# mmechtley/psfMC

Measured on AMD Instinct MI355X. Metric: walker log-posterior evals/sec, 256x256 image, 1 PSF+1 Sersic, higher is better.
Workload: dtype f64

## Files before the change

psfmc_amd/csrc/psfmc_fused_path.h:

```cpp
#pragma once
#ifndef PSFMC_PART
#define PSFMC_PART 0
#endif
#include "psfmc_device.h"
#include "psfmc_fft.h"

#ifndef PSFMC_COLS3G_MIN
#define PSFMC_COLS3G_MIN 0
#endif

namespace psfmc {

#ifndef PSFMC_ROW_WAVES
#define PSFMC_ROW_WAVES 0
#endif
constexpr int kColThreads = 256;
#ifndef PSFMC_COLS_PRIO
#define PSFMC_COLS_PRIO 3
#endif
#ifndef PSFMC_INV_PRIO
#define PSFMC_INV_PRIO 0
#endif
#ifndef PSFMC_INV_REMAP_MIN
#define PSFMC_INV_REMAP_MIN 720
// ... 111 lines not shown
__device__ __forceinline__ int t_elem(int y, int c, int rg_log2) {
    const int rg = 1 << rg_log2;
    return (((y >> rg_log2) * 2 + c) << rg_log2) + (y & (rg - 1));
}
#ifndef PSFMC_T_PAD
#define PSFMC_T_PAD 0
#endif
__host__ __device__ __forceinline__ int t_col_len(int ny, int rg_log2) {
    const int len = ((ny + (1 << rg_log2) - 1) >> rg_log2) << rg_log2;
    return (PSFMC_T_PAD && (len & 127) == 0) ? len + (1 << rg_log2) : len;
}

struct FieldPx {
    double sci, var;
};

template <int NX> constexpr size_t fused_field_len(int ny) {
    return (size_t)((ny + FftShape<NX>::TPW - 1) / FftShape<NX>::TPW) * FftShape<NX>::R * 64;
}

template <int NX>
__global__ void k_pack_field(const double* __restrict__ sci, const double* __restrict__ obs_var,
                             const uint8_t* __restrict__ bad, FieldPx* __restrict__ out, int ny) {
    using S = FftShape<NX>;
    constexpr int T = S::T, R = S::R, RG = S::TPW;
    const int n = (int)fused_field_len<NX>(ny);
    for (int i = blockIdx.x * blockDim.x + threadIdx.x; i < n; i += gridDim.x * blockDim.x) {
        const int lane = i & 63, e = (i >> 6) % R, yg = i / (64 * R);
        const int f = lane / T, t = lane % T;
        const int y = yg * RG + f, x = fft_k_of<NX>(t, e);
        const bool holds = f < RG && y < ny && fft_slot_valid<NX>(t, e);
        const size_t src = holds ? (size_t)y * NX + x : 0;
        out[i] = holds ? FieldPx{bad[src] ? __builtin_nan("") : sci[src], obs_var[src]}
                       : FieldPx{__builtin_nan(""), 1.0};
    }
}

template <int NX, bool FROM_IMAGE, typename TS = cd, bool FAST = FftShape<NX>::kPlain, bool WRAP = false,
          bool EXTRA = false>
__global__ void __launch_bounds__((row_threads<NX, FAST>()), (fused_row_min_waves<NX, false, WRAP>()))
k_rows_fwd(const double* __restrict__ prep, const uint8_t* __restrict__ skip,
           const cd* __restrict__ twx, TS* __restrict__ Tbuf, int n_ps, int n_sersic, int ny,
           int ps_only, const double* __restrict__ img, const double* __restrict__ img_scale,
           double* __restrict__ raw_out, const WrapDesc* __restrict__ wrap_tab, int pow_mode) {
    using S = FftShape<NX>;
    constexpr int P = S::P, T = S::T, R = S::R, RG = row_group<NX>();
    constexpr int NXH = NX / 2 + 1;
    constexpr int RGL2 = layout_rg_log2<NX, FAST>(), RGL = 1 << RGL2;
    extern __shared__ __align__(16) double smem[];
// ... 624 lines not shown
template <class S> constexpr bool cols3f_half_table() { return cols3f_waves<S>() == 8; }
template <class S> constexpr int cols3f_table_rows() { return cols3f_half_table<S>() ? S::R1 / 2 : S::R1; }
template <class S> constexpr size_t fused_col3f_lds_used() {
    return ((size_t)cols3f_waves<S>() * fft3g_lds_doubles<S>() + (size_t)cols3f_table_rows<S>() * 64 * 2) * sizeof(double);
}
template <class S> constexpr size_t fused_col3f_lds_bytes() { return fused_col3f_lds_used<S>(); }
#ifndef PSFMC_COLS3F_PREFETCH
#define PSFMC_COLS3F_PREFETCH -1
#endif
#ifndef PSFMC_COLS3F_WAVES16
#define PSFMC_COLS3F_WAVES16 3
#endif
template <class S> constexpr bool cols3f_prefetch() {
    return PSFMC_COLS3F_PREFETCH < 0 ? (S::R1 == 16 || (S::R1 == 32 && !cols3f_half_table<S>())) : PSFMC_COLS3F_PREFETCH != 0;
}
template <class S> constexpr int cols3f_min_waves() {
    if (cols3f_prefetch<S>()) return S::R1 <= 8 ? 3 : S::R1 <= 16 ? 2 : 1;
    return S::R1 <= 8 ? 4 : S::R1 <= 16 ? PSFMC_COLS3F_WAVES16 : (S::R1 <= 24 || cols3f_half_table<S>()) ? 2 : 1;
}

template <int NY, bool CONVOLVE, class S = Fft3gShape<NY>>
__global__ void __launch_bounds__((cols3f_threads<S>()), (cols3f_min_waves<S>()))
k_cols3f(cd* __restrict__ Tbuf, const cd* __restrict__ Kt, const double* __restrict__ prep,
         const uint8_t* __restrict__ skip, const cd* __restrict__ twy, int plen, int nxh, int n_w, int rg_log2) {
    static_assert(cols3f_shape<S>(), "ny = 8 m x 8 x 8");
    constexpr int R1 = S::R1, NB3 = S::NB3, WPB = cols3f_waves<S>();
    constexpr bool HALF = cols3f_half_table<S>();
    static_assert(NB3 * 8 == R1, "registers");
    static_assert(fused_col3f_lds_bytes<S>() <= 160 * 1024, "a workgroup's LDS");
    extern __shared__ __align__(16) double smem[];
// ... 72 lines not shown
            }
            __builtin_amdgcn_sched_barrier(0);
            fft_wave3g<S, +1, HALF>(v, o, w2, t, lds, tab, w1h);
            __builtin_amdgcn_sched_barrier(0);
            if (live) {
                unsigned os = off_b;
                if constexpr (kScalar) asm volatile("" : "+v"(os));
#pragma unroll
                for (int q = 0; q < NB3; ++q)
#pragma unroll
                    for (int k3 = 0; k3 < 8; ++k3) *t_at(base, os, q + NB3 * k3) = o[q][k3];
            }
        }
        return;
    }
    for (int grp = gr.first; grp < gr.end; grp += gr.step) {
        const int col = grp * WPB + wave;
        if (col >= n_cols) continue;
        const int pr = col >> 1, c = col & 1;
        const int kx = __builtin_amdgcn_readfirstlane(pr / n_w), w = pr - kx * n_w;
        const bool skipped = skip && skip[w];
        cd* base = Tbuf + ((size_t)w * nxh + kx) * 2 * nyp + (c << rg_log2);
        unsigned ob = off_b, kb = kt_b;
        if constexpr (kScalar) asm volatile("" : "+v"(ob), "+v"(kb));
        cd v[R1];
#pragma unroll
        for (int a = 0; a < R1; ++a) v[a] = load_stream(t_at(base, ob, a));
        if (skipped) continue;
        cd o[NB3][8];
        fft_wave3g<S, -1, HALF>(v, o, w2, t, lds, tab, w1h);
        if constexpr (CONVOLVE) {
            __builtin_amdgcn_sched_barrier(0);
            const int psf = __builtin_amdgcn_readfirstlane((int)prep[(size_t)w * plen + kPrepPsfIdx]);
            const cd* k = Kt + (((size_t)psf * nxh + kx) * 2 + c) * NY;
#pragma unroll
            for (int q = 0; q < NB3; ++q)
#pragma unroll
                for (int k3 = 0; k3 < 8; ++k3) v[q + NB3 * k3] = cmul(o[q][k3], *k_at(k, kb, q + NB3 * k3));
            __builtin_amdgcn_sched_barrier(0);
            fft_wave3g<S, +1, HALF>(v, o, w2, t, lds, tab, w1h);
            __builtin_amdgcn_sched_barrier(0);
        }
        unsigned os = off_b;
        if constexpr (kScalar) asm volatile("" : "+v"(os));
#pragma unroll
        for (int q = 0; q < NB3; ++q)
#pragma unroll
            for (int k3 = 0; k3 < 8; ++k3) *t_at(base, os, q + NB3 * k3) = o[q][k3];
    }
}

template <int NX, typename TS = cd, bool FAST = FftShape<NX>::kPlain, bool MULTI = false>
__global__ void __launch_bounds__((row_threads<NX, FAST>()), (fused_row_min_waves<NX, true>()))
k_rows_inv(const TS* __restrict__ Tbuf, const uint8_t* __restrict__ skip, const cd* __restrict__ twx,
           const FieldPx* __restrict__ field, double* __restrict__ partial, int ny,
           const double* __restrict__ prep, int plen,
           double* __restrict__ conv_out, double* __restrict__ var_out, int n_psf_field, unsigned field_stride) {
    using S = FftShape<NX>;
    constexpr int P = S::P, T = S::T, R = S::R, RG = row_group<NX>();
    constexpr int NXH = NX / 2 + 1;
    constexpr int RGL2 = layout_rg_log2<NX, FAST>(), RGL = 1 << RGL2;
    extern __shared__ __align__(16) double smem[];
#if PSFMC_INV_PRIO
    __builtin_amdgcn_s_setprio(PSFMC_INV_PRIO);
#endif

    int w = blockIdx.y, bx = blockIdx.x;
    if constexpr (inv_remap<NX, FAST>()) {
        const int gx = (int)gridDim.x, n_w = (int)gridDim.y;
        const int id = w * gx + bx;
// ... 91 lines not shown
    load_twiddles<NX>(tw, twx, t, twl, lane);
    fft_wave<NX, +1>(v, tw, twx, t, wave_lds + (size_t)fe * fft_lds_elems<NX>(), twl, lane_on);
    const double inv_lambda = prep[(size_t)w * plen + kPrepInvLambda];

    if (conv_out) {
        const size_t rowoff = (size_t)w * ny * NX + (size_t)(row_on ? iy : 0) * NX;
#pragma unroll
        for (int e = 0; e < R; ++e) {
            if (row_on && fft_slot_valid<NX>(t, e)) {
                const int x = fft_k_of<NX>(t, e);
                conv_out[rowoff + x] = v[e].x;
                var_out[rowoff + x] = v[e].y * inv_lambda;
            }
        }
    }
    const FieldPx* fbase = field + (size_t)yg * R * 64;
    if (MULTI || (NX < 1024 && n_psf_field > 0))
        fbase += (size_t)((int)prep[(size_t)w * plen + kPrepPsfIdx] / n_psf_field) * field_stride;
    const unsigned foff = (unsigned)lane * (unsigned)sizeof(FieldPx);
    constexpr int CH = (FAST && R == 32) ? PSFMC_INV_CHUNK : R, NCH = R / CH;
    static_assert(R % CH == 0, "chunks");
    double acc = 0.0, mant = 1.0;
    int expo = 0, n_good = 0;
    bool invalid = false;
    auto load_chunk = [&](FieldPx (&px)[CH], int c) {
#pragma unroll
        for (int j = 0; j < CH; ++j) px[j] = *at_bytes(fbase, foff + (unsigned)((c * CH + j) * 64 * sizeof(FieldPx)));
    };
    auto sum_chunk = [&](const FieldPx (&px)[CH], int c) {
        bool any_bad = false;
#pragma unroll
        for (int j = 0; j < CH; ++j) any_bad |= px[j].sci != px[j].sci;
        if (!__any(any_bad)) {
#pragma unroll
            for (int j = 0; j < CH; ++j) {
                const int e = c * CH + j;
                const double d = __builtin_fma(v[e].y, inv_lambda, px[j].var);
                const double r = px[j].sci - v[e].x;
                acc = __builtin_fma(r * r, fast_rcp(d), acc);
                invalid |= !(d > 0.0);
                mant *= __builtin_amdgcn_frexp_mant(d);
                expo += __builtin_amdgcn_frexp_exp(d);
            }
            n_good += CH;
        } else {
#pragma unroll
            for (int j = 0; j < CH; ++j) {
                const int e = c * CH + j;
                const bool good = px[j].sci == px[j].sci;
                const double d = __builtin_fma(v[e].y, inv_lambda, px[j].var);
                const double r = px[j].sci - v[e].x;
                const double a1 = __builtin_fma(r * r, fast_rcp(d), acc);
                acc = good ? a1 : acc;
                const double dd = good ? d : 1.0;
                invalid |= !(dd > 0.0);
                mant *= __builtin_amdgcn_frexp_mant(dd);
                expo += __builtin_amdgcn_frexp_exp(dd);
                n_good += good ? 1 : 0;
            }
        }
    };
    if constexpr (NCH == 1) {
        FieldPx px[CH];
        load_chunk(px, 0);
        sum_chunk(px, 0);
    } else {
        static_assert(NCH % 2 == 0, "chunk pairs");
        FieldPx pa[CH], pb[CH];
        load_chunk(pa, 0);
#pragma unroll
        for (int c = 0; c < NCH; c += 2) {
            load_chunk(pb, c + 1);
            sum_chunk(pa, c);
            if (c + 2 < NCH) load_chunk(pa, c + 2);
            sum_chunk(pb, c + 1);
        }
    }
    acc += 0.69314718055994530942 * (fast_log2(mant) + (double)expo) +
           1.83787706640934548356 * (double)n_good;
    acc = invalid ? __builtin_nan("") : acc;
#pragma unroll
    for (int o = 32; o > 0; o >>= 1) acc += __shfl_down(acc, o, 64);
    if (lane == 0) partial[(size_t)w * nyg + yg] = acc;
// ... 177 lines not shown
```

psfmc_amd/csrc/psfmc_hip.hip:

```cpp
#include "../../include/psfmc_hip.h"
#include "psfmc_side_costs.h"

#ifndef PSFMC_NPARTS
#define PSFMC_NPARTS 1
#define PSFMC_PART 0
#endif

#include <hip/hip_runtime.h>
#include <hipfft/hipfft.h>

#include <cmath>
#include <cstdarg>
#include <cstdio>
#include <cstdlib>
#include <cstring>
#include <map>
#include <string>
#include <utility>
#include <vector>

#include "psfmc_device.h"
#if PSFMC_PART == 0
#include "psfmc_hipfft_path.h"
#endif
// ... 261 lines not shown
        case 1280: { constexpr int N_ = 1280; BODY; } break; \
        default: return PSFMC_NOT_MINE; \
    }
#endif

struct psfmc_ctx {
    int device = 0;
    int ny = 0, nx = 0, nxh = 0, S = 0, F = 0;
    int nyp = 0;
    bool embed = false;
    std::vector<WrapDesc> wraps;
    WrapDesc* d_wrap = nullptr;
    int n_psf = 0, n_ps = 0, n_sersic = 0;
    int n_fields = 1, n_psf_field = 0;
    size_t field_len = 0;
    int max_walkers = 0, chunk = 0, backend = 0;
    bool prep_tabs_built = false;
    bool prep_tabs_valid = false;
    bool use_pow_tabs = true;
    int single_cap = 0;
    int rlen = 0, plen = 0;
    int nblk = 0;
    hipStream_t stream = nullptr;
    double *d_sci = nullptr, *d_var = nullptr;
    uint8_t* d_bad = nullptr;
    double *d_rows = nullptr, *d_prep = nullptr, *d_like = nullptr, *d_partial = nullptr;
    uint8_t* d_skip = nullptr;
    double2 *d_pspec = nullptr, *d_vspec = nullptr;
    double* d_real = nullptr;
    double2* d_spec = nullptr;
// ... 16 lines not shown
    long long speculated_runs = 0;
    int speculate = -1;
    int cols3 = 1;
    bool use_graph = false;
    long long graph_launches = 0;
    int min_split = 1 << 30;
    bool profile = false;
    struct ProfRec { int kind; hipEvent_t a, b; };
    std::vector<ProfRec> prof_pending;
    double prof_ms[3] = {0, 0, 0};
    long prof_n[3] = {0, 0, 0};
    cd* d_Kraw = nullptr;
    cd* d_Kt = nullptr;
    cd *d_twx = nullptr, *d_twy = nullptr;
    double* d_rho = nullptr;
    FieldPx* d_field = nullptr;
    int rg_log2 = 0;
    double *d_img0 = nullptr, *d_img1 = nullptr;
    int img_cap = 0;
    bool has_layout = false;
    ThetaLayout layout{};
    std::vector<ThetaLayout> more_layouts;
    std::vector<void*> more_blobs;
    std::vector<char> more_has;
    size_t theta_lds = 0;
    ThetaLayout* d_field_layouts = nullptr;
    int* d_field_sides = nullptr;
    void* d_layout_blob = nullptr;
    struct Joint {
        bool ready = false;
        ThetaLayout prior{};
// ... 83 lines not shown
    return PSFMC_OK;
}
template <int NX, bool FROM_IMAGE>
static int launch_rows3_fwd(psfmc_ctx* c, int n, const double* prep, const uint8_t* skip, cd* Tbuf, int ps_only,
                            const double* img, const double* img_scale, double* raw_out, hipStream_t st) {
    if constexpr (!rows3_fwd_built(NX)) {
        return fail(PSFMC_EINVAL, "side %d has no three-stage row kernels", NX);
    } else {
        if constexpr (!FROM_IMAGE) {
            if (c->embed)
                return launch_rows3_fwd_kernel<NX, false, true>(c, n, prep, skip, Tbuf, ps_only, img, img_scale, raw_out, st);
        }
        return launch_rows3_fwd_kernel<NX, FROM_IMAGE, false>(c, n, prep, skip, Tbuf, ps_only, img, img_scale, raw_out, st);
    }
}
template <int NX, bool MULTI>
static int launch_rows3_inv_kernel(psfmc_ctx* c, int n, const cd* Tbuf, const double* prep, const uint8_t* skip,
                                   double* partial, double* conv_out, double* var_out, hipStream_t st) {
    using S = typename Rows3<NX>::S;
    constexpr size_t lds = rows3_lds_bytes<S>();
    if constexpr (lds > 64 * 1024) {
        static thread_local int attr_device = -1;
        if (attr_device != c->device) {
            HIP_TRY(hipFuncSetAttribute(reinterpret_cast<const void*>(&k_rows3_inv<NX, MULTI>),
                                        hipFuncAttributeMaxDynamicSharedMemorySize, (int)lds));
            attr_device = c->device;
        }
    }
    hipLaunchKernelGGL((k_rows3_inv<NX, MULTI>), dim3((c->ny + rows3_waves(NX) - 1) / rows3_waves(NX), n), dim3(rows3_threads(NX)), lds,
                       st, Tbuf, skip, c->d_twx, c->d_field, partial, c->ny, prep, c->plen, conv_out, var_out,
                       c->n_fields > 1 ? c->n_psf_field : 0, (unsigned)c->field_len);
    return PSFMC_OK;
}
template <int NX>
static int launch_rows3_inv(psfmc_ctx* c, int n, const cd* Tbuf, const double* prep, const uint8_t* skip,
                            double* partial, double* conv_out, double* var_out, hipStream_t st) {
    if constexpr (!rows3_side<NX>()) {
        return fail(PSFMC_EINVAL, "side %d has no three-stage row kernels", NX);
    } else {
        if (c->n_fields > 1) return launch_rows3_inv_kernel<NX, true>(c, n, Tbuf, prep, skip, partial, conv_out, var_out, st);
        return launch_rows3_inv_kernel<NX, false>(c, n, Tbuf, prep, skip, partial, conv_out, var_out, st);
    }
}

template <int NX, bool FROM_IMAGE, typename TS, bool FAST, bool WRAP, bool EXTRA = false>
static int launch_rows_fwd_kernel(psfmc_ctx* c, int n, const double* prep, const uint8_t* skip, TS* Tbuf,
                                  int ps_only, const double* img, const double* img_scale, double* raw_out,
                                  hipStream_t st) {
    constexpr size_t lds = fused_row_lds_bytes<NX, FAST>();
    if constexpr (!FROM_IMAGE && !EXTRA) {
        if (const double* extra = ps_only ? nullptr : integ_image_of(c, prep))
            return launch_rows_fwd_kernel<NX, false, TS, FAST, WRAP, true>(c, n, prep, skip, Tbuf, ps_only, extra,
                                                                           img_scale, raw_out, st);
    }
    if constexpr (lds > 64 * 1024) {
        static thread_local int attr_device = -1;
// ... 131 lines not shown
}

template <int NY> static int col_engine_code(const psfmc_ctx* c) {
    if constexpr (cols3f_shape<Fft3gShape<NY>>()) {
        if ((c->cols3 == 1 || c->cols3 == 4) && !c->t_f32) return 3;
    }
    if constexpr (NY == 512 || NY == 1024) {
        if (c->cols3 == 3 || (c->cols3 && c->t_f32)) return 1;
    }
    if constexpr (cols3g_side<NY>()) {
        if (!c->t_f32 && c->cols3 && cols3g_layout_ok<Fft3gShape<NY>>(c->rg_log2)) return 2;
    }
    return 0;
}

template <int NX, typename TS, bool FAST, bool MULTI>
static int launch_rows_inv_kernel(psfmc_ctx* c, int n, const TS* Tbuf, const double* prep, const uint8_t* skip,
                                  double* partial, double* conv_out, double* var_out, hipStream_t st) {
    constexpr size_t lds = fused_row_lds_bytes<NX, FAST>();
    if constexpr (lds > 64 * 1024) {
        static thread_local int attr_device = -1;
        if (attr_device != c->device) {
            HIP_TRY(hipFuncSetAttribute(reinterpret_cast<const void*>(&k_rows_inv<NX, TS, FAST, MULTI>),
                                        hipFuncAttributeMaxDynamicSharedMemorySize, (int)lds));
            attr_device = c->device;
        }
    }
    constexpr int waves = row_waves<NX, FAST>();
    const int gx = (c->nblk + waves - 1) / waves;
    hipLaunchKernelGGL((k_rows_inv<NX, TS, FAST, MULTI>), dim3(gx, n),
                       dim3((row_threads<NX, FAST>())), lds, st, Tbuf, skip, c->d_twx, c->d_field, partial, c->ny,
                       prep, c->plen, conv_out, var_out, c->n_fields > 1 ? c->n_psf_field : 0, (unsigned)c->field_len);
    return PSFMC_OK;
}

template <int NX, typename TS, bool FAST>
static int launch_rows_inv_impl(psfmc_ctx* c, int n, const TS* Tbuf, const double* prep, const uint8_t* skip,
                                double* partial, double* conv_out, double* var_out, hipStream_t st) {
    if constexpr (sizeof(TS) == sizeof(cd) && NX >= 1024) {
        if (c->n_fields > 1)
            return launch_rows_inv_kernel<NX, TS, FAST, true>(c, n, Tbuf, prep, skip, partial, conv_out, var_out, st);
    } else if constexpr (sizeof(TS) != sizeof(cd)) {
        if (c->n_fields > 1) return fail(PSFMC_EINVAL, "single-precision storage serves contexts of one field");
    }
    return launch_rows_inv_kernel<NX, TS, FAST, false>(c, n, Tbuf, prep, skip, partial, conv_out, var_out, st);
}

template <int NX, typename TS = cd>
// ... 9 lines not shown
            if (c->rows3_inv)
                return launch_rows3_inv<NX>(c, n, static_cast<const cd*>(Tvoid), prep, skip, partial, conv_out, var_out, st);
        }
        if constexpr (FftShape<NX>::kPlain) {
            if (c->row_fast)
                return launch_rows_inv_impl<NX, TS, true>(c, n, Tbuf, prep, skip, partial, conv_out, var_out, st);
        }
        if constexpr (sizeof(TS) == sizeof(cd)) {
            return launch_rows_inv_impl<NX, TS, false>(c, n, Tbuf, prep, skip, partial, conv_out, var_out, st);
        } else {
            return fail(PSFMC_EINVAL, "single-precision storage needs the unguarded row kernels");
        }
    }
}

template <int NX> static int pack_field(psfmc_ctx* c, int f) {
    const size_t px = (size_t)f * c->S;
    if constexpr (rows3_side<NX>()) {
        if (c->rows3_inv) {
            hipLaunchKernelGGL((k_pack_field3<NX>), dim3(256), dim3(256), 0, c->stream, c->d_sci + px, c->d_var + px,
                               c->d_bad + px, c->d_field + (size_t)f * c->field_len, c->ny);
            return PSFMC_OK;
        }
    }
    if constexpr (two_stage_side(NX)) {
        hipLaunchKernelGGL((k_pack_field<NX>), dim3(256), dim3(256), 0, c->stream, c->d_sci + px, c->d_var + px,
                           c->d_bad + px, c->d_field + (size_t)f * c->field_len, c->ny);
        return PSFMC_OK;
    } else {
        return fail(PSFMC_EINVAL, "side %d needs the three-stage row kernels", NX);
    }
}
template <int NX> static RowShape row_shape_of(bool rows3) {
    if constexpr (rows3_side<NX>()) {
        if (rows3 || !two_stage_side(NX)) return RowShape{1, rows3_waves(NX), rows3_rg_log2(NX), Rows3<NX>::S::R1, false};
    }
    if constexpr (two_stage_side(NX))
        return RowShape{row_group<NX>(), row_waves<NX, true>(), layout_rg_log2<NX, true>(), FftShape<NX>::R,
                        FftShape<NX>::kPlain};
    else
        return RowShape{1, rows3_waves(NX), rows3_rg_log2(NX), 0, false};
}
template <int NX> constexpr int row_families() {
    return (two_stage_side(NX) ? 1 : 0) | (rows3_side<NX>() ? 2 : 0) | (rows3_fwd_built(NX) ? 4 : 0) |
           (rows3_side<NX>() && rows3_inv_default(NX) ? 8 : 0);
}
// ... 310 lines not shown
        RC_TRY(size_call(SZ_ROWS_FWD, c->nx, a));
        a.convolve = false;
        RC_TRY(size_call(SZ_COLS, c->ny, a));
    }
    hipLaunchKernelGGL(k_scale_kernel_spectrum, dim3(256), dim3(256), 0, c->stream, c->d_Kraw, c->d_Kt,
                       (int)n_el, c->ny, c->nxh, c->rg_log2, 0.25 / (double)c->S);
    HIP_TRY(hipGetLastError());
    HIP_TRY(hipStreamSynchronize(c->stream));
    return PSFMC_OK;
}

extern "C" int psfmc_abi_version(void) { return 1; }

extern "C" const char* psfmc_last_error(void) { return g_err.c_str(); }

static int ctx_init(psfmc_ctx* c, const double* sci, const double* obs_var, const uint8_t* bad_px,
                    const int* psf_ny, const int* psf_nx, const double* psf, const double* psf_var) {
    HIP_TRY(hipStreamCreateWithFlags(&c->stream, hipStreamNonBlocking));
    HIP_TRY(hipEventCreateWithFlags(&c->ev_fork, hipEventDisableTiming));
    for (int i = 0; i < psfmc_ctx::kMaxStreams; ++i) HIP_TRY(hipEventCreateWithFlags(&c->ev_stagger[i], hipEventDisableTiming));
    for (int k = 0; k < 3; ++k)
        for (int i = 0; i < 2; ++i) HIP_TRY(hipEventCreateWithFlags(&c->ev_excl[k][i], hipEventDisableTiming));
    for (int i = 1; i < psfmc_ctx::kMaxStreams; ++i) {
        HIP_TRY(hipStreamCreateWithFlags(&c->side[i], hipStreamNonBlocking));
        HIP_TRY(hipEventCreateWithFlags(&c->ev_join[i], hipEventDisableTiming));
    }
    const size_t all_px = (size_t)c->n_fields * c->S;
    HIP_TRY(hipMalloc(&c->d_sci, all_px * sizeof(double)));
    HIP_TRY(hipMalloc(&c->d_var, all_px * sizeof(double)));
    HIP_TRY(hipMalloc(&c->d_bad, all_px));
// ... 38 lines not shown
            if (tot > 0.0 && std::isfinite(tot)) {
                int e;
                (void)frexp(tot, &e);
                rho[p] = ldexp(1.0, -e);
            }
        }
        HIP_TRY(hipMalloc(&c->d_rho, c->n_psf * sizeof(double)));
        HIP_TRY(hipMemcpy(c->d_rho, rho.data(), c->n_psf * sizeof(double), hipMemcpyHostToDevice));
        size_t field_len = 0;
        {
            SizeCall a;
            a.len = &field_len; a.ny = c->ny; a.rows3 = c->rows3_inv;
            RC_TRY(size_call(SZ_FIELD_LEN, c->nx, a));
        }
        c->field_len = field_len;
        HIP_TRY(hipMalloc(&c->d_field, (size_t)c->n_fields * field_len * sizeof(FieldPx)));
        for (int f = 0; f < c->n_fields; ++f) {
            SizeCall a;
            a.c = c; a.field = f;
            RC_TRY(size_call(SZ_PACK_FIELD, c->nx, a));
        }
    }

    std::vector<double> inter(2 * psf_off[c->n_fields]);
    for (int p = 0; p < c->n_psf; ++p) {
        const int f = p / c->n_psf_field;
        const size_t small = (size_t)psf_ny[f] * psf_nx[f];
        const size_t src = psf_off[f] + (size_t)(p % c->n_psf_field) * small;
        const size_t dst = 2 * psf_off[f] + (size_t)(2 * (p % c->n_psf_field)) * small;
        memcpy(&inter[dst], psf + src, small * sizeof(double));
        memcpy(&inter[dst + small], psf_var + src, small * sizeof(double));
    }
    double *d_small = nullptr, *d_canvas = nullptr;
    HIP_TRY(hipMalloc(&d_small, inter.size() * sizeof(double)));
    int rc = PSFMC_OK;
    if (hipMalloc(&d_canvas, (size_t)2 * c->n_psf * c->S * sizeof(double)) != hipSuccess)
// ... 315 lines not shown
    if (!strcmp(key, "storage_f32")) {
        const bool on = value != 0;
        if (on && (c->backend != PSFMC_BACKEND_FUSED || !c->plain_shape || !c->row_fast || c->embed))
            return fail(PSFMC_EINVAL, "storage_f32 needs the fused back end and power-of-two sides");
        HIP_TRY(hipSetDevice(c->device));
        HIP_TRY(hipDeviceSynchronize());
        c->t_f32 = on;
        c->chunk = fused_pass_walkers(c);
        if (c->chunk > c->max_walkers) c->chunk = c->max_walkers;
        if (c->d_img0) { (void)hipFree(c->d_img0); c->d_img0 = nullptr; }
        if (c->d_img1) { (void)hipFree(c->d_img1); c->d_img1 = nullptr; }
        if (c->d_rawstage) { (void)hipFree(c->d_rawstage); c->d_rawstage = nullptr; }
        c->img_cap = 0;
        return alloc_work(c);
    }
    if (!strcmp(key, "cols_grid")) {
        if (value < 1) return fail(PSFMC_EINVAL, "cols_grid must be >= 1");
        c->cols_grid = (int)value;
        return PSFMC_OK;
    }
    if (!strcmp(key, "stagger")) {
        c->stagger = (int)value;
        return PSFMC_OK;
    }
    if (!strcmp(key, "exclusive")) {
        c->exclusive = (int)value & 7;
        return PSFMC_OK;
    }
    if (!strcmp(key, "linear_accumulation")) {
        HIP_TRY(hipSetDevice(c->device));
// ... 55 lines not shown
    if (!strcmp(key, "column_engine")) {
        if (c->backend != PSFMC_BACKEND_FUSED) return NAN;
        int code = 0;
        SizeCall a;
        a.c = c; a.code = &code;
        return size_call(SZ_COL_ENGINE, c->ny, a) == PSFMC_OK ? (double)code : NAN;
    }
    if (!strcmp(key, "speculate")) return c->speculate;
    if (!strcmp(key, "pow_tabs")) return c->use_pow_tabs ? 1.0 : 0.0;
    if (!strcmp(key, "pow_tabs_built")) return c->prep_tabs_built ? 1.0 : 0.0;
    if (!strcmp(key, "speculated_runs")) return (double)c->speculated_runs;
    if (!strcmp(key, "transform_ny")) return c->ny;
    if (!strcmp(key, "transform_nx")) return c->nx;
    if (!strcmp(key, "partials_per_walker")) return c->nblk;
    if (!strcmp(key, "storage_f32")) return c->t_f32 ? 1.0 : 0.0;
    if (!strcmp(key, "graph_launches")) return (double)c->graph_launches;
    if (!strcmp(key, "chunk_walkers")) return c->chunk;
    if (!strcmp(key, "backend")) return c->backend;
    if (!strcmp(key, "max_walkers")) return c->max_walkers;
    if (!strcmp(key, "cols_grid")) return c->cols_grid;
    if (!strcmp(key, "streams")) return c->n_streams;
    if (!strcmp(key, "stagger")) return c->stagger;
    if (!strcmp(key, "exclusive")) return c->exclusive;
    if (!strcmp(key, "cols3")) return c->cols3;
    if (!strcmp(key, "linear_accumulation")) return c->linear_acc ? 1.0 : 0.0;
    return NAN;
}

static int hipfft_convolve(psfmc_ctx* c, int n, const double* d_prep, const uint8_t* d_skip,
                           hipStream_t st, int ps_only) {
// ... 1872 lines not shown
```

psfmc_amd/csrc/psfmc_rows3_path.h:

```cpp
#pragma once
#include "psfmc_fused_path.h"

namespace psfmc {

#ifndef PSFMC_ROWS3_WAVES_2048
#define PSFMC_ROWS3_WAVES_2048 8
#endif
#ifndef PSFMC_ROWS3_WAVES_1280
#define PSFMC_ROWS3_WAVES_1280 4
#endif
constexpr int rows3_waves(int n) { return n == 2048 ? PSFMC_ROWS3_WAVES_2048 : n == 1280 ? PSFMC_ROWS3_WAVES_1280 : 4; }
constexpr int rows3_threads(int n) { return 64 * rows3_waves(n); }
#ifndef PSFMC_ROWS3_HALF_1152
#define PSFMC_ROWS3_HALF_1152 1
#endif
#ifndef PSFMC_ROWS3_HALF_1280
#define PSFMC_ROWS3_HALF_1280 0
#endif
constexpr bool rows3_half_table(int n) {
    return (n == 2048 && rows3_waves(n) == 8) || (PSFMC_ROWS3_HALF_1152 && n == 1152) || (PSFMC_ROWS3_HALF_1280 && n == 1280);
}
template <class S> constexpr int rows3_table_rows() { return rows3_half_table(S::kN) ? S::R1 / 2 : S::R1; }
#ifndef PSFMC_ROWS3_BIG_RG_LOG2
#define PSFMC_ROWS3_BIG_RG_LOG2 0
// ... 53 lines not shown
template <class S, bool INVERSE> constexpr int rows3_min_waves() {
    return S::R1 <= 8 ? 4 : S::R1 <= 16 ? PSFMC_ROWS3_WAVES16 : (S::R1 <= 24 || rows3_waves(S::kN) > 4) ? 2 : 1;
}
#ifndef PSFMC_ROWS3_RASTER_GROUP
#define PSFMC_ROWS3_RASTER_GROUP 1
#endif
#ifndef PSFMC_ROWS3_PREFETCH
#define PSFMC_ROWS3_PREFETCH 0
#endif
#ifndef PSFMC_DEBUG_ROWS3
#define PSFMC_DEBUG_ROWS3 0
#endif

template <int NX> constexpr size_t rows3_field_len(int ny) { return (size_t)ny * Rows3<NX>::NSLOT * 64; }

template <int NX>
__global__ void k_pack_field3(const double* __restrict__ sci, const double* __restrict__ obs_var,
                              const uint8_t* __restrict__ bad, FieldPx* __restrict__ out, int ny) {
    using S = typename Rows3<NX>::S;
    constexpr int NSLOT = Rows3<NX>::NSLOT;
    const size_t n = rows3_field_len<NX>(ny);
    for (size_t i = (size_t)blockIdx.x * blockDim.x + threadIdx.x; i < n; i += (size_t)gridDim.x * blockDim.x) {
        const int lane = (int)(i & 63), e = (int)((i >> 6) % NSLOT), y = (int)(i / (64 * NSLOT));
        const int q = e / S::R3, k3 = e % S::R3;
        const bool holds = fft3g_valid<S>(lane, q);
        const size_t src = holds ? (size_t)y * NX + fft3g_index<S>(lane, q, k3) : 0;
        out[i] = holds ? FieldPx{bad[src] ? __builtin_nan("") : sci[src], obs_var[src]}
                       : FieldPx{__builtin_nan(""), 1.0};
    }
}

__device__ __forceinline__ double swap_adjacent_lanes(double v) {
    const long long b = __builtin_bit_cast(long long, v);
    int lo = (int)b, hi = (int)(b >> 32);
    lo = __builtin_amdgcn_update_dpp(lo, lo, 0xB1, 0xF, 0xF, false);
    hi = __builtin_amdgcn_update_dpp(hi, hi, 0xB1, 0xF, 0xF, false);
    return __builtin_bit_cast(double, ((long long)hi << 32) | (long long)(unsigned)lo);
}
__device__ __forceinline__ cd pair_trade(bool odd, cd from_even, cd from_odd) {
    const double sx = odd ? from_odd.x : from_even.x, sy = odd ? from_odd.y : from_even.y;
    return cd{swap_adjacent_lanes(sx), swap_adjacent_lanes(sy)};
}
__device__ __forceinline__ cd pick(bool second, cd a, cd b) { return cd{second ? b.x : a.x, second ? b.y : a.y}; }
// ... 154 lines not shown
#pragma unroll
        for (int k3 = 0; k3 < R3; ++k3) {
            const int k = fft3g_index<S>(t, q, k3);
            if (fft3g_valid<S>(t, q) && 2 * k <= NX) {
                const cd zk = o[q][k3];
                const bool self = k == 0 || 2 * k == NX;
                cd zm = ubuf[self ? 1 : k];
                if (self) zm = zk;
                cd* dst = at_bytes(wbase, off_row + (unsigned)k * kstride);
                dst[0] = cd{zk.x + zm.x, zk.y - zm.y};
                dst[RGL] = cd{zk.y + zm.y, zm.x - zk.x};
            }
        }
}

template <int NX, bool MULTI = false, class S = typename Rows3<NX>::S>
__global__ void __launch_bounds__((rows3_threads(NX)), (rows3_min_waves<S, true>()))
k_rows3_inv(const cd* __restrict__ Tbuf, const uint8_t* __restrict__ skip, const cd* __restrict__ twx,
            const FieldPx* __restrict__ field, double* __restrict__ partial, int ny,
            const double* __restrict__ prep, int plen, double* __restrict__ conv_out, double* __restrict__ var_out,
            int n_psf_field, unsigned field_stride) {
    constexpr int R1 = S::R1, R2 = S::R2, R3 = S::R3, L = S::L, NB3 = S::NB3, NSLOT = NB3 * R3;
    constexpr int RGL2 = rows3_rg_log2(NX), NXH = NX / 2 + 1, RGL = 1 << RGL2;
    constexpr int WAVES = rows3_waves(NX);
    constexpr bool kPair = RGL2 == 0 && L == 64;
    extern __shared__ __align__(16) double smem[];
    int w = blockIdx.y, bx = blockIdx.x;
    {
        const int gx = (int)gridDim.x, n_w = (int)gridDim.y;
        const int id = w * gx + bx;
        const int WB = n_w <= kInvRemapMaxWalkers ? n_w : 8;
        const int B = id / (WB * gx), rem = id - B * WB * gx;
        const int left = n_w - B * WB, wb = left < WB ? left : WB;
        const int q8 = gx & ~7;
// ... 74 lines not shown
    cd o[NB3][R3];
    fft_wave3g<S, +1, rows3_half_table(NX)>(v, o, w2, t, wave_lds, tab, twx[(R1 / 2) * tl]);
    const double inv_lambda = prep[(size_t)w * plen + kPrepInvLambda];
    if (conv_out) {
        const size_t rowoff = (size_t)w * ny * NX + (size_t)iy * NX;
#pragma unroll
        for (int q = 0; q < NB3; ++q)
#pragma unroll
            for (int k3 = 0; k3 < R3; ++k3)
                if (fft3g_valid<S>(t, q)) {
                    const int x = fft3g_index<S>(t, q, k3);
                    conv_out[rowoff + x] = o[q][k3].x;
                    var_out[rowoff + x] = o[q][k3].y * inv_lambda;
                }
    }
    const FieldPx* fbase = field + (size_t)iy * NSLOT * 64;
    if (MULTI || n_psf_field > 0)
        fbase += (size_t)((int)prep[(size_t)w * plen + kPrepPsfIdx] / (n_psf_field > 0 ? n_psf_field : 1)) * field_stride;
    const unsigned foff = (unsigned)t * (unsigned)sizeof(FieldPx);
    constexpr int CH = NSLOT % 16 == 0 ? 8 : NSLOT, NCH = NSLOT / CH;
    double acc = 0.0, mant = 1.0;
    int expo = 0, n_good = 0;
    bool invalid = false;
    auto load_chunk = [&](FieldPx (&px)[CH], int c) {
#pragma unroll
        for (int j = 0; j < CH; ++j) px[j] = *at_bytes(fbase, foff + (unsigned)((c * CH + j) * 64 * sizeof(FieldPx)));
    };
    auto sum_chunk = [&](const FieldPx (&px)[CH], int c) {
        bool any_bad = false;
#pragma unroll
        for (int j = 0; j < CH; ++j) any_bad |= px[j].sci != px[j].sci;
        if (!__any(any_bad)) {
#pragma unroll
            for (int j = 0; j < CH; ++j) {
                const int e = c * CH + j;
                const cd z = o[e / R3][e % R3];
                const double d = __builtin_fma(z.y, inv_lambda, px[j].var);
                const double r = px[j].sci - z.x;
                acc = __builtin_fma(r * r, fast_rcp(d), acc);
                invalid |= !(d > 0.0);
                mant *= __builtin_amdgcn_frexp_mant(d);
                expo += __builtin_amdgcn_frexp_exp(d);
            }
            n_good += CH;
        } else {
#pragma unroll
            for (int j = 0; j < CH; ++j) {
                const int e = c * CH + j;
                const cd z = o[e / R3][e % R3];
                const bool good = px[j].sci == px[j].sci;
                const double d = __builtin_fma(z.y, inv_lambda, px[j].var);
                const double r = px[j].sci - z.x;
                const double a1 = __builtin_fma(r * r, fast_rcp(d), acc);
                acc = good ? a1 : acc;
                const double dd = good ? d : 1.0;
                invalid |= !(dd > 0.0);
                mant *= __builtin_amdgcn_frexp_mant(dd);
                expo += __builtin_amdgcn_frexp_exp(dd);
                n_good += good ? 1 : 0;
            }
        }
    };
    if constexpr (NCH == 1) {
        FieldPx px[CH];
        load_chunk(px, 0);
        sum_chunk(px, 0);
    } else {
        static_assert(NCH % 2 == 0, "chunk pairs");
        FieldPx pa[CH], pb[CH];
        load_chunk(pa, 0);
#pragma unroll
        for (int c = 0; c < NCH; c += 2) {
            load_chunk(pb, c + 1);
            sum_chunk(pa, c);
            if (c + 2 < NCH) load_chunk(pa, c + 2);
            sum_chunk(pb, c + 1);
        }
    }
    acc += 0.69314718055994530942 * (fast_log2(mant) + (double)expo) +
           1.83787706640934548356 * (double)n_good;
    acc = invalid ? __builtin_nan("") : acc;
#pragma unroll
    for (int off = 32; off > 0; off >>= 1) acc += __shfl_down(acc, off, 64);
    if (t == 0) partial[(size_t)w * ny + iy] = acc;
// ... 4 lines not shown
```

Before: 1.409 million.

## Store packed sci/var field as float32 when lossless; add cols3f store barrier

Adds a float32 packed form of the science/variance field that is used automatically when every value round-trips exactly through float, halving the bytes the inverse-row likelihood kernels read per pixel. Values are widened back to double before the likelihood arithmetic, so results stay the same. It also adds an optional path in the column convolve kernel for the 32-radix shape that runs a workgroup barrier before the stores, so waves write back together, with out-of-range waves clamped instead of skipped. The cost is an extra host scan of the inputs at init, plus added template variants.

```diff
diff --git a/psfmc_amd/csrc/psfmc_fused_path.h b/psfmc_amd/csrc/psfmc_fused_path.h
--- a/psfmc_amd/csrc/psfmc_fused_path.h
+++ b/psfmc_amd/csrc/psfmc_fused_path.h
@@ -149,14 +149,21 @@
 struct FieldPx {
     double sci, var;
 };
+struct alignas(8) FieldPxF {
+    float sci, var;
+};
+template <typename PX> __device__ __forceinline__ PX make_field_px(double sci, double var) {
+    using V = decltype(PX::sci);
+    return PX{(V)sci, (V)var};
+}
 
 template <int NX> constexpr size_t fused_field_len(int ny) {
     return (size_t)((ny + FftShape<NX>::TPW - 1) / FftShape<NX>::TPW) * FftShape<NX>::R * 64;
 }
 
-template <int NX>
+template <int NX, typename PX>
 __global__ void k_pack_field(const double* __restrict__ sci, const double* __restrict__ obs_var,
-                             const uint8_t* __restrict__ bad, FieldPx* __restrict__ out, int ny) {
+                             const uint8_t* __restrict__ bad, PX* __restrict__ out, int ny) {
     using S = FftShape<NX>;
     constexpr int T = S::T, R = S::R, RG = S::TPW;
     const int n = (int)fused_field_len<NX>(ny);
@@ -166,8 +173,8 @@
         const int y = yg * RG + f, x = fft_k_of<NX>(t, e);
         const bool holds = f < RG && y < ny && fft_slot_valid<NX>(t, e);
         const size_t src = holds ? (size_t)y * NX + x : 0;
-        out[i] = holds ? FieldPx{bad[src] ? __builtin_nan("") : sci[src], obs_var[src]}
-                       : FieldPx{__builtin_nan(""), 1.0};
+        out[i] = holds ? make_field_px<PX>(bad[src] ? __builtin_nan("") : sci[src], obs_var[src])
+                       : make_field_px<PX>(__builtin_nan(""), 1.0);
     }
 }
 
@@ -822,6 +829,12 @@
 template <class S> constexpr bool cols3f_prefetch() {
     return PSFMC_COLS3F_PREFETCH < 0 ? (S::R1 == 16 || (S::R1 == 32 && !cols3f_half_table<S>())) : PSFMC_COLS3F_PREFETCH != 0;
 }
+#ifndef PSFMC_COLS3F_STORE_MEET
+#define PSFMC_COLS3F_STORE_MEET 1
+#endif
+template <class S> constexpr bool cols3f_store_meet() {
+    return PSFMC_COLS3F_STORE_MEET != 0 && S::R1 == 32 && !cols3f_prefetch<S>();
+}
 template <class S> constexpr int cols3f_min_waves() {
     if (cols3f_prefetch<S>()) return S::R1 <= 8 ? 3 : S::R1 <= 16 ? 2 : 1;
     return S::R1 <= 8 ? 4 : S::R1 <= 16 ? PSFMC_COLS3F_WAVES16 : (S::R1 <= 24 || cols3f_half_table<S>()) ? 2 : 1;
@@ -924,9 +937,12 @@
         }
         return;
     }
+    constexpr bool kMeet = cols3f_store_meet<S>() && CONVOLVE;
     for (int grp = gr.first; grp < gr.end; grp += gr.step) {
-        const int col = grp * WPB + wave;
-        if (col >= n_cols) continue;
+        int col = grp * WPB + wave;
+        const bool inside = col < n_cols;
+        if constexpr (kMeet) col = inside ? col : n_cols - 1;
+        else if (!inside) continue;
         const int pr = col >> 1, c = col & 1;
         const int kx = __builtin_amdgcn_readfirstlane(pr / n_w), w = pr - kx * n_w;
         const bool skipped = skip && skip[w];
@@ -936,6 +952,33 @@
         cd v[R1];
 #pragma unroll
         for (int a = 0; a < R1; ++a) v[a] = load_stream(t_at(base, ob, a));
+        if constexpr (kMeet) {
+            const bool run = inside && !skipped;
+            cd o[NB3][8];
+            if (run) {
+                fft_wave3g<S, -1, HALF>(v, o, w2, t, lds, tab, w1h);
+                __builtin_amdgcn_sched_barrier(0);
+                const int psf = __builtin_amdgcn_readfirstlane((int)prep[(size_t)w * plen + kPrepPsfIdx]);
+                const cd* k = Kt + (((size_t)psf * nxh + kx) * 2 + c) * NY;
+#pragma unroll
+                for (int q = 0; q < NB3; ++q)
+#pragma unroll
+                    for (int k3 = 0; k3 < 8; ++k3) v[q + NB3 * k3] = cmul(o[q][k3], *k_at(k, kb, q + NB3 * k3));
+                __builtin_amdgcn_sched_barrier(0);
+                fft_wave3g<S, +1, HALF>(v, o, w2, t, lds, tab, w1h);
+                __builtin_amdgcn_sched_barrier(0);
+            }
+            __builtin_amdgcn_s_barrier();
+            if (run) {
+                unsigned os = off_b;
+                if constexpr (kScalar) asm volatile("" : "+v"(os));
+#pragma unroll
+                for (int q = 0; q < NB3; ++q)
+#pragma unroll
+                    for (int k3 = 0; k3 < 8; ++k3) *t_at(base, os, q + NB3 * k3) = o[q][k3];
+            }
+            continue;
+        }
         if (skipped) continue;
         cd o[NB3][8];
         fft_wave3g<S, -1, HALF>(v, o, w2, t, lds, tab, w1h);
@@ -960,10 +1003,10 @@
     }
 }
 
-template <int NX, typename TS = cd, bool FAST = FftShape<NX>::kPlain, bool MULTI = false>
+template <int NX, typename TS = cd, bool FAST = FftShape<NX>::kPlain, bool MULTI = false, typename PX = FieldPx>
 __global__ void __launch_bounds__((row_threads<NX, FAST>()), (fused_row_min_waves<NX, true>()))
 k_rows_inv(const TS* __restrict__ Tbuf, const uint8_t* __restrict__ skip, const cd* __restrict__ twx,
-           const FieldPx* __restrict__ field, double* __restrict__ partial, int ny,
+           const PX* __restrict__ field, double* __restrict__ partial, int ny,
            const double* __restrict__ prep, int plen,
            double* __restrict__ conv_out, double* __restrict__ var_out, int n_psf_field, unsigned field_stride) {
     using S = FftShape<NX>;
@@ -1085,20 +1128,23 @@
             }
         }
     }
-    const FieldPx* fbase = field + (size_t)yg * R * 64;
+    const PX* fbase = field + (size_t)yg * R * 64;
     if (MULTI || (NX < 1024 && n_psf_field > 0))
         fbase += (size_t)((int)prep[(size_t)w * plen + kPrepPsfIdx] / n_psf_field) * field_stride;
-    const unsigned foff = (unsigned)lane * (unsigned)sizeof(FieldPx);
+    const unsigned foff = (unsigned)lane * (unsigned)sizeof(PX);
     constexpr int CH = (FAST && R == 32) ? PSFMC_INV_CHUNK : R, NCH = R / CH;
     static_assert(R % CH == 0, "chunks");
     double acc = 0.0, mant = 1.0;
     int expo = 0, n_good = 0;
     bool invalid = false;
-    auto load_chunk = [&](FieldPx (&px)[CH], int c) {
-#pragma unroll
-        for (int j = 0; j < CH; ++j) px[j] = *at_bytes(fbase, foff + (unsigned)((c * CH + j) * 64 * sizeof(FieldPx)));
+    auto load_chunk = [&](PX (&px)[CH], int c) {
+#pragma unroll
+        for (int j = 0; j < CH; ++j) px[j] = *at_bytes(fbase, foff + (unsigned)((c * CH + j) * 64 * sizeof(PX)));
     };
-    auto sum_chunk = [&](const FieldPx (&px)[CH], int c) {
+    auto sum_chunk = [&](const PX (&raw)[CH], int c) {
+        FieldPx px[CH];
+#pragma unroll
+        for (int j = 0; j < CH; ++j) px[j] = FieldPx{(double)raw[j].sci, (double)raw[j].var};
         bool any_bad = false;
 #pragma unroll
         for (int j = 0; j < CH; ++j) any_bad |= px[j].sci != px[j].sci;
@@ -1106,8 +1152,9 @@
 #pragma unroll
             for (int j = 0; j < CH; ++j) {
                 const int e = c * CH + j;
-                const double d = __builtin_fma(v[e].y, inv_lambda, px[j].var);
-                const double r = px[j].sci - v[e].x;
+                const double sci = px[j].sci, var = px[j].var;
+                const double d = __builtin_fma(v[e].y, inv_lambda, var);
+                const double r = sci - v[e].x;
                 acc = __builtin_fma(r * r, fast_rcp(d), acc);
                 invalid |= !(d > 0.0);
                 mant *= __builtin_amdgcn_frexp_mant(d);
@@ -1119,8 +1166,9 @@
             for (int j = 0; j < CH; ++j) {
                 const int e = c * CH + j;
                 const bool good = px[j].sci == px[j].sci;
-                const double d = __builtin_fma(v[e].y, inv_lambda, px[j].var);
-                const double r = px[j].sci - v[e].x;
+                const double sci = px[j].sci, var = px[j].var;
+                const double d = __builtin_fma(v[e].y, inv_lambda, var);
+                const double r = sci - v[e].x;
                 const double a1 = __builtin_fma(r * r, fast_rcp(d), acc);
                 acc = good ? a1 : acc;
                 const double dd = good ? d : 1.0;
@@ -1132,12 +1180,12 @@
         }
     };
     if constexpr (NCH == 1) {
-        FieldPx px[CH];
+        PX px[CH];
         load_chunk(px, 0);
         sum_chunk(px, 0);
     } else {
         static_assert(NCH % 2 == 0, "chunk pairs");
-        FieldPx pa[CH], pb[CH];
+        PX pa[CH], pb[CH];
         load_chunk(pa, 0);
 #pragma unroll
         for (int c = 0; c < NCH; c += 2) {
diff --git a/psfmc_amd/csrc/psfmc_hip.hip b/psfmc_amd/csrc/psfmc_hip.hip
--- a/psfmc_amd/csrc/psfmc_hip.hip
+++ b/psfmc_amd/csrc/psfmc_hip.hip
@@ -299,6 +299,9 @@
     int n_psf = 0, n_ps = 0, n_sersic = 0;
     int n_fields = 1, n_psf_field = 0;
     size_t field_len = 0;
+    int field_f32_req = -1;
+    bool field_fits_f32 = false;
+    bool field_f32 = false;
     int max_walkers = 0, chunk = 0, backend = 0;
     bool prep_tabs_built = false;
     bool prep_tabs_valid = false;
@@ -345,7 +348,7 @@
     cd* d_Kt = nullptr;
     cd *d_twx = nullptr, *d_twy = nullptr;
     double* d_rho = nullptr;
-    FieldPx* d_field = nullptr;
+    void* d_field = nullptr;
     int rg_log2 = 0;
     double *d_img0 = nullptr, *d_img1 = nullptr;
     int img_cap = 0;
@@ -459,7 +462,7 @@
         return launch_rows3_fwd_kernel<NX, FROM_IMAGE, false>(c, n, prep, skip, Tbuf, ps_only, img, img_scale, raw_out, st);
     }
 }
-template <int NX, bool MULTI>
+template <int NX, bool MULTI, typename PX>
 static int launch_rows3_inv_kernel(psfmc_ctx* c, int n, const cd* Tbuf, const double* prep, const uint8_t* skip,
                                    double* partial, double* conv_out, double* var_out, hipStream_t st) {
     using S = typename Rows3<NX>::S;
@@ -467,13 +470,13 @@
     if constexpr (lds > 64 * 1024) {
         static thread_local int attr_device = -1;
         if (attr_device != c->device) {
-            HIP_TRY(hipFuncSetAttribute(reinterpret_cast<const void*>(&k_rows3_inv<NX, MULTI>),
+            HIP_TRY(hipFuncSetAttribute(reinterpret_cast<const void*>(&k_rows3_inv<NX, MULTI, PX>),
                                         hipFuncAttributeMaxDynamicSharedMemorySize, (int)lds));
             attr_device = c->device;
         }
     }
-    hipLaunchKernelGGL((k_rows3_inv<NX, MULTI>), dim3((c->ny + rows3_waves(NX) - 1) / rows3_waves(NX), n), dim3(rows3_threads(NX)), lds,
-                       st, Tbuf, skip, c->d_twx, c->d_field, partial, c->ny, prep, c->plen, conv_out, var_out,
+    hipLaunchKernelGGL((k_rows3_inv<NX, MULTI, PX>), dim3((c->ny + rows3_waves(NX) - 1) / rows3_waves(NX), n), dim3(rows3_threads(NX)), lds,
+                       st, Tbuf, skip, c->d_twx, static_cast<const PX*>(c->d_field), partial, c->ny, prep, c->plen, conv_out, var_out,
                        c->n_fields > 1 ? c->n_psf_field : 0, (unsigned)c->field_len);
     return PSFMC_OK;
 }
@@ -483,8 +486,12 @@
     if constexpr (!rows3_side<NX>()) {
         return fail(PSFMC_EINVAL, "side %d has no three-stage row kernels", NX);
     } else {
-        if (c->n_fields > 1) return launch_rows3_inv_kernel<NX, true>(c, n, Tbuf, prep, skip, partial, conv_out, var_out, st);
-        return launch_rows3_inv_kernel<NX, false>(c, n, Tbuf, prep, skip, partial, conv_out, var_out, st);
+        if (c->field_f32) {
+            if (c->n_fields > 1) return launch_rows3_inv_kernel<NX, true, FieldPxF>(c, n, Tbuf, prep, skip, partial, conv_out, var_out, st);
+            return launch_rows3_inv_kernel<NX, false, FieldPxF>(c, n, Tbuf, prep, skip, partial, conv_out, var_out, st);
+        }
+        if (c->n_fields > 1) return launch_rows3_inv_kernel<NX, true, FieldPx>(c, n, Tbuf, prep, skip, partial, conv_out, var_out, st);
+        return launch_rows3_inv_kernel<NX, false, FieldPx>(c, n, Tbuf, prep, skip, partial, conv_out, var_out, st);
     }
 }
 
@@ -646,24 +653,32 @@
     return 0;
 }
 
-template <int NX, typename TS, bool FAST, bool MULTI>
-static int launch_rows_inv_kernel(psfmc_ctx* c, int n, const TS* Tbuf, const double* prep, const uint8_t* skip,
+template <int NX, typename TS, bool FAST, bool MULTI, typename PX>
+static int launch_rows_inv_kernel_px(psfmc_ctx* c, int n, const TS* Tbuf, const double* prep, const uint8_t* skip,
                                   double* partial, double* conv_out, double* var_out, hipStream_t st) {
     constexpr size_t lds = fused_row_lds_bytes<NX, FAST>();
     if constexpr (lds > 64 * 1024) {
         static thread_local int attr_device = -1;
         if (attr_device != c->device) {
-            HIP_TRY(hipFuncSetAttribute(reinterpret_cast<const void*>(&k_rows_inv<NX, TS, FAST, MULTI>),
+            HIP_TRY(hipFuncSetAttribute(reinterpret_cast<const void*>(&k_rows_inv<NX, TS, FAST, MULTI, PX>),
                                         hipFuncAttributeMaxDynamicSharedMemorySize, (int)lds));
             attr_device = c->device;
         }
     }
     constexpr int waves = row_waves<NX, FAST>();
     const int gx = (c->nblk + waves - 1) / waves;
-    hipLaunchKernelGGL((k_rows_inv<NX, TS, FAST, MULTI>), dim3(gx, n),
-                       dim3((row_threads<NX, FAST>())), lds, st, Tbuf, skip, c->d_twx, c->d_field, partial, c->ny,
-                       prep, c->plen, conv_out, var_out, c->n_fields > 1 ? c->n_psf_field : 0, (unsigned)c->field_len);
-    return PSFMC_OK;
+    hipLaunchKernelGGL((k_rows_inv<NX, TS, FAST, MULTI, PX>), dim3(gx, n),
+                       dim3((row_threads<NX, FAST>())), lds, st, Tbuf, skip, c->d_twx, static_cast<const PX*>(c->d_field),
+                       partial, c->ny, prep, c->plen, conv_out, var_out, c->n_fields > 1 ? c->n_psf_field : 0,
+                       (unsigned)c->field_len);
+    return PSFMC_OK;
+}
+template <int NX, typename TS, bool FAST, bool MULTI>
+static int launch_rows_inv_kernel(psfmc_ctx* c, int n, const TS* Tbuf, const double* prep, const uint8_t* skip,
+                                  double* partial, double* conv_out, double* var_out, hipStream_t st) {
+    if (c->field_f32)
+        return launch_rows_inv_kernel_px<NX, TS, FAST, MULTI, FieldPxF>(c, n, Tbuf, prep, skip, partial, conv_out, var_out, st);
+    return launch_rows_inv_kernel_px<NX, TS, FAST, MULTI, FieldPx>(c, n, Tbuf, prep, skip, partial, conv_out, var_out, st);
 }
 
 template <int NX, typename TS, bool FAST>
@@ -703,22 +718,26 @@
     }
 }
 
-template <int NX> static int pack_field(psfmc_ctx* c, int f) {
+template <int NX, typename PX> static int pack_field_px(psfmc_ctx* c, int f) {
     const size_t px = (size_t)f * c->S;
+    PX* out = static_cast<PX*>(c->d_field) + (size_t)f * c->field_len;
     if constexpr (rows3_side<NX>()) {
         if (c->rows3_inv) {
-            hipLaunchKernelGGL((k_pack_field3<NX>), dim3(256), dim3(256), 0, c->stream, c->d_sci + px, c->d_var + px,
-                               c->d_bad + px, c->d_field + (size_t)f * c->field_len, c->ny);
+            hipLaunchKernelGGL((k_pack_field3<NX, PX>), dim3(256), dim3(256), 0, c->stream, c->d_sci + px, c->d_var + px,
+                               c->d_bad + px, out, c->ny);
             return PSFMC_OK;
         }
     }
     if constexpr (two_stage_side(NX)) {
-        hipLaunchKernelGGL((k_pack_field<NX>), dim3(256), dim3(256), 0, c->stream, c->d_sci + px, c->d_var + px,
-                           c->d_bad + px, c->d_field + (size_t)f * c->field_len, c->ny);
+        hipLaunchKernelGGL((k_pack_field<NX, PX>), dim3(256), dim3(256), 0, c->stream, c->d_sci + px, c->d_var + px,
+                           c->d_bad + px, out, c->ny);
         return PSFMC_OK;
     } else {
         return fail(PSFMC_EINVAL, "side %d needs the three-stage row kernels", NX);
     }
+}
+template <int NX> static int pack_field(psfmc_ctx* c, int f) {
+    return c->field_f32 ? pack_field_px<NX, FieldPxF>(c, f) : pack_field_px<NX, FieldPx>(c, f);
 }
 template <int NX> static RowShape row_shape_of(bool rows3) {
     if constexpr (rows3_side<NX>()) {
@@ -1059,6 +1078,29 @@
 
 extern "C" const char* psfmc_last_error(void) { return g_err.c_str(); }
 
+static bool field_fits_f32(const double* sci, const double* obs_var, const uint8_t* bad_px, size_t n) {
+    for (size_t i = 0; i < n; ++i) {
+        const double s = sci[i], v = obs_var[i];
+        if (!((double)(float)v == v)) return false;
+        if (!(bad_px[i] || s != s || (double)(float)s == s)) return false;
+    }
+    return true;
+}
+
+static int pack_fields(psfmc_ctx* c) {
+    const bool family = c->rows3_inv || (c->plain_shape && c->row_fast);
+    c->field_f32 = c->field_fits_f32 && (c->field_f32_req == 1 || (c->field_f32_req < 0 && family));
+    if (c->d_field) { (void)hipFree(c->d_field); c->d_field = nullptr; }
+    HIP_TRY(hipMalloc(&c->d_field, (size_t)c->n_fields * c->field_len * (c->field_f32 ? sizeof(FieldPxF) : sizeof(FieldPx))));
+    for (int f = 0; f < c->n_fields; ++f) {
+        SizeCall a;
+        a.c = c; a.field = f;
+        RC_TRY(size_call(SZ_PACK_FIELD, c->nx, a));
+    }
+    HIP_TRY(hipGetLastError());
+    return PSFMC_OK;
+}
+
 static int ctx_init(psfmc_ctx* c, const double* sci, const double* obs_var, const uint8_t* bad_px,
                     const int* psf_ny, const int* psf_nx, const double* psf, const double* psf_var) {
     HIP_TRY(hipStreamCreateWithFlags(&c->stream, hipStreamNonBlocking));
@@ -1127,12 +1169,8 @@
             RC_TRY(size_call(SZ_FIELD_LEN, c->nx, a));
         }
         c->field_len = field_len;
-        HIP_TRY(hipMalloc(&c->d_field, (size_t)c->n_fields * field_len * sizeof(FieldPx)));
-        for (int f = 0; f < c->n_fields; ++f) {
-            SizeCall a;
-            a.c = c; a.field = f;
-            RC_TRY(size_call(SZ_PACK_FIELD, c->nx, a));
-        }
+        c->field_fits_f32 = field_fits_f32(sci, obs_var, bad_px, all_px);
+        RC_TRY(pack_fields(c));
     }
 
     std::vector<double> inter(2 * psf_off[c->n_fields]);
@@ -1478,6 +1516,24 @@
         c->img_cap = 0;
         return alloc_work(c);
     }
+    if (!strcmp(key, "field_f32")) {
+        if (!(value == -1 || value == 0 || value == 1))
+            return fail(PSFMC_EINVAL, "field_f32 must be -1 (automatic), 0 or 1 (got %g)", value);
+        if (c->backend != PSFMC_BACKEND_FUSED) {
+            if (value == 1) return fail(PSFMC_EINVAL, "field_f32 = 1 needs the fused back end");
+            c->field_f32_req = (int)value;
+            return PSFMC_OK;
+        }
+        if (value == 1 && !c->field_fits_f32)
+            return fail(PSFMC_EINVAL, "field_f32 = 1: a sci or obs_var value of this context is not a float32 "
+                        "number, the packed form would change it");
+        HIP_TRY(hipSetDevice(c->device));
+        HIP_TRY(hipDeviceSynchronize());
+        c->field_f32_req = (int)value;
+        RC_TRY(pack_fields(c));
+        HIP_TRY(hipStreamSynchronize(c->stream));
+        return PSFMC_OK;
+    }
     if (!strcmp(key, "cols_grid")) {
         if (value < 1) return fail(PSFMC_EINVAL, "cols_grid must be >= 1");
         c->cols_grid = (int)value;
@@ -1563,6 +1619,8 @@
     if (!strcmp(key, "transform_nx")) return c->nx;
     if (!strcmp(key, "partials_per_walker")) return c->nblk;
     if (!strcmp(key, "storage_f32")) return c->t_f32 ? 1.0 : 0.0;
+    if (!strcmp(key, "field_f32")) return c->field_f32_req;
+    if (!strcmp(key, "field_f32_active")) return c->field_f32 ? 1.0 : 0.0;
     if (!strcmp(key, "graph_launches")) return (double)c->graph_launches;
     if (!strcmp(key, "chunk_walkers")) return c->chunk;
     if (!strcmp(key, "backend")) return c->backend;
diff --git a/psfmc_amd/csrc/psfmc_rows3_path.h b/psfmc_amd/csrc/psfmc_rows3_path.h
--- a/psfmc_amd/csrc/psfmc_rows3_path.h
+++ b/psfmc_amd/csrc/psfmc_rows3_path.h
@@ -91,9 +91,9 @@
 
 template <int NX> constexpr size_t rows3_field_len(int ny) { return (size_t)ny * Rows3<NX>::NSLOT * 64; }
 
-template <int NX>
+template <int NX, typename PX>
 __global__ void k_pack_field3(const double* __restrict__ sci, const double* __restrict__ obs_var,
-                              const uint8_t* __restrict__ bad, FieldPx* __restrict__ out, int ny) {
+                              const uint8_t* __restrict__ bad, PX* __restrict__ out, int ny) {
     using S = typename Rows3<NX>::S;
     constexpr int NSLOT = Rows3<NX>::NSLOT;
     const size_t n = rows3_field_len<NX>(ny);
@@ -102,8 +102,8 @@
         const int q = e / S::R3, k3 = e % S::R3;
         const bool holds = fft3g_valid<S>(lane, q);
         const size_t src = holds ? (size_t)y * NX + fft3g_index<S>(lane, q, k3) : 0;
-        out[i] = holds ? FieldPx{bad[src] ? __builtin_nan("") : sci[src], obs_var[src]}
-                       : FieldPx{__builtin_nan(""), 1.0};
+        out[i] = holds ? make_field_px<PX>(bad[src] ? __builtin_nan("") : sci[src], obs_var[src])
+                       : make_field_px<PX>(__builtin_nan(""), 1.0);
     }
 }
 
@@ -288,10 +288,10 @@
         }
 }
 
-template <int NX, bool MULTI = false, class S = typename Rows3<NX>::S>
+template <int NX, bool MULTI = false, typename PX = FieldPx, class S = typename Rows3<NX>::S>
 __global__ void __launch_bounds__((rows3_threads(NX)), (rows3_min_waves<S, true>()))
 k_rows3_inv(const cd* __restrict__ Tbuf, const uint8_t* __restrict__ skip, const cd* __restrict__ twx,
-            const FieldPx* __restrict__ field, double* __restrict__ partial, int ny,
+            const PX* __restrict__ field, double* __restrict__ partial, int ny,
             const double* __restrict__ prep, int plen, double* __restrict__ conv_out, double* __restrict__ var_out,
             int n_psf_field, unsigned field_stride) {
     constexpr int R1 = S::R1, R2 = S::R2, R3 = S::R3, L = S::L, NB3 = S::NB3, NSLOT = NB3 * R3;
@@ -396,19 +396,22 @@
                     var_out[rowoff + x] = o[q][k3].y * inv_lambda;
                 }
     }
-    const FieldPx* fbase = field + (size_t)iy * NSLOT * 64;
+    const PX* fbase = field + (size_t)iy * NSLOT * 64;
     if (MULTI || n_psf_field > 0)
         fbase += (size_t)((int)prep[(size_t)w * plen + kPrepPsfIdx] / (n_psf_field > 0 ? n_psf_field : 1)) * field_stride;
-    const unsigned foff = (unsigned)t * (unsigned)sizeof(FieldPx);
+    const unsigned foff = (unsigned)t * (unsigned)sizeof(PX);
     constexpr int CH = NSLOT % 16 == 0 ? 8 : NSLOT, NCH = NSLOT / CH;
     double acc = 0.0, mant = 1.0;
     int expo = 0, n_good = 0;
     bool invalid = false;
-    auto load_chunk = [&](FieldPx (&px)[CH], int c) {
-#pragma unroll
-        for (int j = 0; j < CH; ++j) px[j] = *at_bytes(fbase, foff + (unsigned)((c * CH + j) * 64 * sizeof(FieldPx)));
+    auto load_chunk = [&](PX (&px)[CH], int c) {
+#pragma unroll
+        for (int j = 0; j < CH; ++j) px[j] = *at_bytes(fbase, foff + (unsigned)((c * CH + j) * 64 * sizeof(PX)));
     };
-    auto sum_chunk = [&](const FieldPx (&px)[CH], int c) {
+    auto sum_chunk = [&](const PX (&raw)[CH], int c) {
+        FieldPx px[CH];
+#pragma unroll
+        for (int j = 0; j < CH; ++j) px[j] = FieldPx{(double)raw[j].sci, (double)raw[j].var};
         bool any_bad = false;
 #pragma unroll
         for (int j = 0; j < CH; ++j) any_bad |= px[j].sci != px[j].sci;
@@ -417,8 +420,9 @@
             for (int j = 0; j < CH; ++j) {
                 const int e = c * CH + j;
                 const cd z = o[e / R3][e % R3];
-                const double d = __builtin_fma(z.y, inv_lambda, px[j].var);
-                const double r = px[j].sci - z.x;
+                const double sci = px[j].sci, var = px[j].var;
+                const double d = __builtin_fma(z.y, inv_lambda, var);
+                const double r = sci - z.x;
                 acc = __builtin_fma(r * r, fast_rcp(d), acc);
                 invalid |= !(d > 0.0);
                 mant *= __builtin_amdgcn_frexp_mant(d);
@@ -431,8 +435,9 @@
                 const int e = c * CH + j;
                 const cd z = o[e / R3][e % R3];
                 const bool good = px[j].sci == px[j].sci;
-                const double d = __builtin_fma(z.y, inv_lambda, px[j].var);
-                const double r = px[j].sci - z.x;
+                const double sci = px[j].sci, var = px[j].var;
+                const double d = __builtin_fma(z.y, inv_lambda, var);
+                const double r = sci - z.x;
                 const double a1 = __builtin_fma(r * r, fast_rcp(d), acc);
                 acc = good ? a1 : acc;
                 const double dd = good ? d : 1.0;
@@ -444,12 +449,12 @@
         }
     };
     if constexpr (NCH == 1) {
-        FieldPx px[CH];
+        PX px[CH];
         load_chunk(px, 0);
         sum_chunk(px, 0);
     } else {
         static_assert(NCH % 2 == 0, "chunk pairs");
-        FieldPx pa[CH], pb[CH];
+        PX pa[CH], pb[CH];
         load_chunk(pa, 0);
 #pragma unroll
         for (int c = 0; c < NCH; c += 2) {
```

Result: no change. 1.411 million, median of 2 (+0.1%).
